# sheepTnT/Stage-IndexOrganized

Hardware: AMD Instinct MI355X
Metric: YCSB ops/sec at 1/2/4/8 GPU + achieved HBM GB/s vs peak; CPU ref ops/sec (higher is better)
Workload: dtype u64; 1 GPU; YCSB-C 100M rows uint64 keys, zipf 0.9, batched point-lookup on 1×MI355X; traversal=device, rows_per_gpu=100000000, rows_total=100000000, batch_per_gpu=16777216, key_bytes=8, payload_bytes=1000, leaf_bytes=65536, parallelism=single GPU

## Files before the change

stage-indexorganized_amd/csrc/capi.cpp:

```cpp
#include <hip/hip_runtime_api.h>

#include <execinfo.h>
#include <unistd.h>

#include <csignal>
#include <cstdlib>
#include <cstring>
#include <memory>
#include <stdexcept>
#include <string>
#include <vector>

#include "handle.hpp"

namespace stage_capi {
thread_local std::string g_err;
}
using namespace stage_capi;

extern "C" {

const char *stage_last_error(void) { return g_err.c_str(); }

namespace {
// ... 564 lines not shown
    if (rc) return rc;
    if (n && (!d_start_keys || !d_counts || (!d_records && scan_size))) return fail(STAGE_E_ARG, "null device buffer");
    hipError_t e = hipSetDevice(t->dev.device);
    if (e != hipSuccess) return hip_rc(e, "hipSetDevice");
    e = stage::launch_scan(t->dev.view, d_start_keys, d_lens, n, scan_size, d_counts, d_records, pick(t, stream),
                          t->scan_tune);
    return hip_rc(e, "scan kernel");
}

int stage_index_scan_batch(stage_table *t, const uint64_t *d_start_keys, const uint16_t *d_lens,
                           const uint32_t *d_read_ids, uint64_t n, uint32_t scan_size, uint32_t *d_counts,
                           uint8_t *d_records, uint8_t *d_row_status, void *stream) {
    int rc = need_synced(t);
    if (rc) return rc;
    if (n && (!d_start_keys || !d_counts || (scan_size && (!d_records || !d_row_status))))
        return fail(STAGE_E_ARG, "null device buffer");
    hipError_t e = hipSetDevice(t->dev.device);
    if (e != hipSuccess) return hip_rc(e, "hipSetDevice");
    e = stage::launch_scan(t->dev.view, d_start_keys, d_lens, n, scan_size, d_counts, d_records, pick(t, stream),
                           t->scan_tune, d_read_ids, d_row_status);
    return hip_rc(e, "index scan kernel");
}

static int scan_window(stage_table *t, const uint64_t *d_start_keys, const uint16_t *d_lens, const uint32_t *d_read_ids,
                       uint64_t n, uint32_t scan_size, uint32_t payload_off, uint32_t len, uint32_t *d_counts,
                       uint8_t *d_window, uint8_t *d_row_keys, uint8_t *d_row_status, bool index, void *stream) {
    int rc = check_window(t, payload_off, len);
    if (rc) return rc;
    if (n && scan_size && (!d_start_keys || !d_counts || !d_window || (index && !d_row_status)))
        return fail(STAGE_E_ARG, "null device buffer");
    rc = need_synced(t);
    if (rc) return rc;
    if (n == 0) return STAGE_OK;
    hipError_t e = hipSetDevice(t->dev.device);
    if (e != hipSuccess) return hip_rc(e, "hipSetDevice");
    e = stage::launch_scan_window(t->dev.view, d_start_keys, d_lens, n, scan_size, facts(t).key_pad() + payload_off, len,
                                  facts(t).key_pad(), d_counts, d_window, d_row_keys, pick(t, stream), t->scan_tune,
                                  index ? d_read_ids : nullptr, index ? d_row_status : nullptr);
    return hip_rc(e, index ? "window index scan kernel" : "window scan kernel");
}

int stage_scan_batch_window(stage_table *t, const uint64_t *d_start_keys, const uint16_t *d_lens, uint64_t n,
                            uint32_t scan_size, uint32_t payload_off, uint32_t len, uint32_t *d_counts,
                            uint8_t *d_window, uint8_t *d_row_keys, void *stream) {
    return scan_window(t, d_start_keys, d_lens, nullptr, n, scan_size, payload_off, len, d_counts, d_window, d_row_keys,
                       nullptr, false, stream);
}

int stage_index_scan_batch_window(stage_table *t, const uint64_t *d_start_keys, const uint16_t *d_lens,
                                  const uint32_t *d_read_ids, uint64_t n, uint32_t scan_size, uint32_t payload_off,
                                  uint32_t len, uint32_t *d_counts, uint8_t *d_window, uint8_t *d_row_keys,
                                  uint8_t *d_row_status, void *stream) {
    return scan_window(t, d_start_keys, d_lens, d_read_ids, n, scan_size, payload_off, len, d_counts, d_window,
                       d_row_keys, d_row_status, true, stream);
}

static int table_scan(stage_table *t, uint64_t leaf_begin, uint64_t leaf_end, const uint32_t *read_id, bool window,
                      uint32_t payload_off, uint32_t len, uint64_t max_records, uint64_t *d_count,
                      uint64_t *d_leaf_offsets, uint8_t *d_out, uint8_t *d_row_keys, uint64_t *d_row_meta,
                      uint8_t *d_row_status, void *stream) {
    if (!t) return fail(STAGE_E_ARG, "null table");
    int rc = window ? check_window(t, payload_off, len) : STAGE_OK;
    if (rc) return rc;
    if (leaf_begin > leaf_end) return fail(STAGE_E_ARG, "table scan: leaf_begin exceeds leaf_end");
    if (!d_count) return fail(STAGE_E_ARG, "table scan: null d_count");
    if (max_records && !d_out) return fail(STAGE_E_ARG, "table scan: null record buffer with max_records != 0");
    rc = need_synced(t);
    if (rc) return rc;
    const uint64_t nleaves = t->dev.view.nleaves;
    if (leaf_end == UINT64_MAX) leaf_end = nleaves;
    if (leaf_end > nleaves || leaf_begin > leaf_end)
        return fail(STAGE_E_ARG, "table scan: the leaf range exceeds the table's " + std::to_string(nleaves) + " leaves");
    return guarded([&] {
        hipError_t e = hipSetDevice(t->dev.device);
        if (e != hipSuccess) return hip_rc(e, "hipSetDevice");
        const uint32_t nl = (uint32_t)(leaf_end - leaf_begin);
        uint8_t *scratch = nl ? stage::scratch_bytes(t->dev, stage::table_scan_scratch_bytes(nl)) : nullptr;
        const stage::TableScanOut o{max_records, d_count, d_leaf_offsets, window ? nullptr : d_out,
                                    window ? d_out : nullptr, window ? d_row_keys : nullptr, d_row_meta, d_row_status};
        e = stage::launch_table_scan(t->dev.view, (uint32_t)leaf_begin, nl, read_id != nullptr, read_id ? *read_id : 0u,
                                     window ? facts(t).key_pad() + payload_off : 0u, window ? len : 0u,
                                     facts(t).key_pad(), o, scratch, pick(t, stream), t->scan_tune);
        return hip_rc(e, "table scan kernels");
    });
}

int stage_table_scan(stage_table *t, uint64_t leaf_begin, uint64_t leaf_end, const uint32_t *read_id,
                     uint64_t max_records, uint64_t *d_count, uint64_t *d_leaf_offsets, uint8_t *d_records,
                     uint64_t *d_row_meta, uint8_t *d_row_status, void *stream) {
    return table_scan(t, leaf_begin, leaf_end, read_id, false, 0, 0, max_records, d_count, d_leaf_offsets, d_records,
                      nullptr, d_row_meta, d_row_status, stream);
}

int stage_table_scan_window(stage_table *t, uint64_t leaf_begin, uint64_t leaf_end, const uint32_t *read_id,
                            uint32_t payload_off, uint32_t len, uint64_t max_records, uint64_t *d_count,
                            uint64_t *d_leaf_offsets, uint8_t *d_window, uint8_t *d_row_keys, uint64_t *d_row_meta,
                            uint8_t *d_row_status, void *stream) {
    return table_scan(t, leaf_begin, leaf_end, read_id, true, payload_off, len, max_records, d_count, d_leaf_offsets,
                      d_window, d_row_keys, d_row_meta, d_row_status, stream);
}

int stage_index_scan_first_batch(stage_table *t, const uint64_t *d_start_keys, const uint32_t *d_read_ids,
                                 uint64_t n, uint32_t scan_size, uint32_t prefix_words, uint32_t *d_image,
                                 uint8_t *d_status, void *stream) {
    int rc = need_synced(t);
    if (rc) return rc;
    if (t->dev.view.key_width == 0) return fail(STAGE_E_ARG, "first-tuple scans need fixed-width keys");
    if (scan_size == 0 || scan_size > 63) return fail(STAGE_E_ARG, "scan_size must be 1..63");
    if (prefix_words > t->dev.view.key_words) return fail(STAGE_E_ARG, "prefix_words exceeds the key's words");
    if (n && (!d_start_keys || !d_image || !d_status)) return fail(STAGE_E_ARG, "null device buffer");
    hipError_t e = hipSetDevice(t->dev.device);
    if (e != hipSuccess) return hip_rc(e, "hipSetDevice");
    e = stage::launch_scan_first(t->dev.view, d_start_keys, n, scan_size, d_read_ids, prefix_words, d_image, d_status,
                                 pick(t, stream), t->scan_tune);
    return hip_rc(e, "first-tuple scan kernel");
}

int stage_resolve_batch(stage_table *t, const uint64_t *d_keys, const uint16_t *d_lens, uint64_t n, int le_child,
                        uint32_t *d_leaf, void *stream) {
    int rc = need_synced(t);
    if (rc) return rc;
    if (n && (!d_keys || !d_leaf)) return fail(STAGE_E_ARG, "null device buffer");
    hipError_t e = hipSetDevice(t->dev.device);
    if (e != hipSuccess) return hip_rc(e, "hipSetDevice");
    e = stage::launch_resolve(t->dev.view, d_keys, d_lens, n, le_child, d_leaf, pick(t, stream));
    return hip_rc(e, "resolve kernel");
}

int stage_set_probe_tuning(stage_table *t, int group, int max_blocks) {
    if (!t || (group != 1 && group != 2 && group != 4 && group != 8) || max_blocks < 0)
        return fail(STAGE_E_ARG, "bad tuning");
    t->tune.group = group;
    t->tune.max_blocks = max_blocks;
    return STAGE_OK;
}

int stage_set_scan_tuning(stage_table *t, int max_blocks) {
    if (!t || max_blocks < 0) return fail(STAGE_E_ARG, "bad tuning");
    t->scan_tune.max_blocks = max_blocks;
    return STAGE_OK;
}

int stage_set_probe_store(stage_table *t, int policy) {
    if (!t || policy < STAGE_STORE_TEMPORAL || policy > STAGE_STORE_WRITE_THROUGH)
        return fail(STAGE_E_ARG, "bad store policy");
    t->tune.store = policy;
    return STAGE_OK;
}

int stage_set_probe_form(stage_table *t, int form) {
    if (!t || (form != STAGE_PROBE_FORM_WAVE && form != STAGE_PROBE_FORM_LANE))
        return fail(STAGE_E_ARG, "bad probe form");
    t->tune.form = form;
    return STAGE_OK;
}

int stage_murmur64a_batch(const void *d_keys, uint32_t key_len, uint32_t key_stride, uint64_t seed, uint64_t n,
                          uint64_t *d_out, void *stream) {
    if (n && (!d_keys || !d_out || key_stride < key_len)) return fail(STAGE_E_ARG, "bad arguments");
    return hip_rc(stage::launch_murmur(d_keys, key_len, key_stride, seed, n, d_out, (hipStream_t)stream),
                  "murmur kernel");
}

int stage_set_device(int device) { return hip_rc(hipSetDevice(device), "hipSetDevice"); }
int stage_device_count(int *count) { return hip_rc(hipGetDeviceCount(count), "hipGetDeviceCount"); }
int stage_dev_alloc(uint64_t bytes, void **ptr) { return hip_rc(hipMalloc(ptr, bytes ? bytes : 16), "hipMalloc"); }
int stage_dev_free(void *ptr) { return hip_rc(hipFree(ptr), "hipFree"); }
int stage_dev_memset(void *ptr, int value, uint64_t bytes, void *stream) {
    return hip_rc(hipMemsetAsync(ptr, value, bytes, (hipStream_t)stream), "hipMemsetAsync");
}
int stage_memcpy_h2d(void *dst, const void *src, uint64_t bytes, void *stream) {
    hipError_t e = hipMemcpyAsync(dst, src, bytes, hipMemcpyHostToDevice, (hipStream_t)stream);
    if (e == hipSuccess) e = hipStreamSynchronize((hipStream_t)stream);
    return hip_rc(e, "h2d");
}
int stage_memcpy_d2h(void *dst, const void *src, uint64_t bytes, void *stream) {
    hipError_t e = hipMemcpyAsync(dst, src, bytes, hipMemcpyDeviceToHost, (hipStream_t)stream);
    if (e == hipSuccess) e = hipStreamSynchronize((hipStream_t)stream);
    return hip_rc(e, "d2h");
}
int stage_stream_create(void **stream) {
    return hip_rc(hipStreamCreateWithFlags((hipStream_t *)stream, hipStreamNonBlocking), "hipStreamCreate");
}
int stage_stream_destroy(void *stream) { return hip_rc(hipStreamDestroy((hipStream_t)stream), "hipStreamDestroy"); }
int stage_stream_sync(void *stream) { return hip_rc(hipStreamSynchronize((hipStream_t)stream), "hipStreamSynchronize"); }
int stage_device_sync(void) { return hip_rc(hipDeviceSynchronize(), "hipDeviceSynchronize"); }
int stage_event_create(void **ev) { return hip_rc(hipEventCreate((hipEvent_t *)ev), "hipEventCreate"); }
int stage_event_destroy(void *ev) { return hip_rc(hipEventDestroy((hipEvent_t)ev), "hipEventDestroy"); }
int stage_event_record(void *ev, void *stream) {
    return hip_rc(hipEventRecord((hipEvent_t)ev, (hipStream_t)stream), "hipEventRecord");
}
int stage_event_elapsed(void *a, void *b, float *ms) {
    hipError_t e = hipEventSynchronize((hipEvent_t)b);
    if (e == hipSuccess) e = hipEventElapsedTime(ms, (hipEvent_t)a, (hipEvent_t)b);
    return hip_rc(e, "hipEventElapsedTime");
}

int stage_comm_unique_id(uint8_t *id128) {
    if (!id128) return fail(STAGE_E_ARG, "null argument");
    return guarded([&] { return stage::shard_unique_id(id128); });
}

int stage_comm_init(stage_table *t, const uint8_t *id128, int rank, int world) {
    if (!t || !id128 || world < 1 || rank < 0 || rank >= world) return fail(STAGE_E_ARG, "bad arguments");
    if (facts(t).key_words() != 1) return fail(STAGE_E_ARG, "the sharded front-end routes keys of <= 8 bytes");
    return guarded([&] {
        (void)hipSetDevice(t->dev.device);
        t->comm = std::make_unique<stage::ShardComm>();
        const int rc = stage::shard_init(*t->comm, id128, rank, world, t->shard_chunks);
        if (t->shard_dedupe >= 0) t->comm->dedupe = t->shard_dedupe != 0;
        t->comm->key_bits = t->shard_key_bits;
        return rc;
    });
}

int stage_set_shard_dedupe(stage_table *t, int on) {
    if (!t || on < -1 || on > 1) return fail(STAGE_E_ARG, "dedupe must be -1, 0 or 1");
    t->shard_dedupe = on;
    const bool v = on < 0 ? stage::shard_default_dedupe() : on != 0;
    if (t->comm) t->comm->dedupe = v;
    if (t->loop_comm) t->loop_comm->dedupe = v;
    return STAGE_OK;
}

int stage_set_write_overlap(stage_table *t, int on) {
    if (!t || on < 0 || on > 1) return fail(STAGE_E_ARG, "write overlap must be 0 or 1");
    t->wp_overlap = on;
    return STAGE_OK;
}

int stage_set_shard_key_bits(stage_table *t, int bits) {
    if (!t || bits < 0 || bits > 64) return fail(STAGE_E_ARG, "bits must be 0..64");
    t->shard_key_bits = bits ? bits : 64;
    if (t->comm) t->comm->key_bits = t->shard_key_bits;
    if (t->loop_comm) t->loop_comm->key_bits = t->shard_key_bits;
    return STAGE_OK;
}

int stage_rccl_info(int *runtime_version, int *header_version, char *path, uint64_t path_len) {
    return guarded([&] { return stage::shard_rccl_info(runtime_version, header_version, path, path_len); });
}

int stage_sharded_stats(stage_table *t, int loopback, uint64_t *n_keys, uint64_t *n_routed, uint64_t *n_remote) {
    if (!t || !n_keys || !n_routed || !n_remote) return fail(STAGE_E_ARG, "null argument");
    stage::ShardComm *c = loopback ? t->loop_comm.get() : t->comm.get();
    if (!c) return fail(STAGE_E_STATE, "no sharded probe has run");
    *n_keys = c->last_n;
    *n_routed = c->last_routed;
    *n_remote = c->last_remote;
    return STAGE_OK;
}

int stage_sharded_stats_ex(stage_table *t, int loopback, uint64_t *v, int nv) {
    if (!t || !v || nv < 0) return fail(STAGE_E_ARG, "bad arguments");
    stage::ShardComm *c = loopback ? t->loop_comm.get() : t->comm.get();
    if (!c) return fail(STAGE_E_STATE, "no sharded probe has run");
    const uint64_t all[4] = {c->last_n, c->last_routed, c->last_remote, c->last_received};
    for (int i = 0; i < nv && i < 4; ++i) v[i] = all[i];
    return STAGE_OK;
}

int stage_comm_allreduce_f64(stage_table *t, double *values, uint64_t n, int op) {
    if (!t || (!values && n) || op < 0 || op > 2) return fail(STAGE_E_ARG, "bad arguments");
    if (!t->comm) return fail(STAGE_E_STATE, "stage_comm_init first");
    return guarded([&] {
        (void)hipSetDevice(t->dev.device);
        return stage::shard_allreduce_f64(*t->comm, values, n, op);
    });
}

int stage_comm_allgather_f64(stage_table *t, const double *in, uint64_t n, double *out) {
    if (!t || ((!in || !out) && n)) return fail(STAGE_E_ARG, "bad arguments");
    if (!t->comm) return fail(STAGE_E_STATE, "stage_comm_init first");
    return guarded([&] {
        (void)hipSetDevice(t->dev.device);
        return stage::shard_allgather_f64(*t->comm, in, n, out);
    });
}

int stage_set_shard_chunks(stage_table *t, int chunks) {
    if (!t || chunks < 0 || chunks > 64) return fail(STAGE_E_ARG, "chunks must be 0..64");
    t->shard_chunks = chunks;
    return STAGE_OK;
}

int stage_comm_destroy(stage_table *t) {
    if (!t) return fail(STAGE_E_ARG, "null table");
    return guarded([&] {
        t->comm.reset();
        return STAGE_OK;
    });
}

int stage_probe_sharded(stage_table *t, const uint64_t *d_keys, const uint32_t *d_read_ids, uint64_t n,
                        stage_probe_out *d_out, uint8_t *d_records, void *stream) {
    int rc = need_synced(t);
    if (rc) return rc;
    if (!t->comm) return fail(STAGE_E_STATE, "stage_comm_init first");
    return guarded([&] {
        (void)hipSetDevice(t->dev.device);
        stage::DevTable view = t->dev.view;
        if (t->out_stride) view.stride = t->out_stride;
        return stage::shard_probe(*t->comm, view, t->tune, d_keys, d_read_ids, n,
                                  reinterpret_cast<stage::stage_probe_out_dev *>(d_out), d_records, STAGE_REPLY_ROWS,
                                  pick(t, stream));
    });
// ... 84 lines not shown
```

stage-indexorganized_amd/csrc/kernel_api.hpp:

```cpp
#pragma once
#include <hip/hip_runtime_api.h>

#include <cstdint>

#include "stage_core.hpp"

namespace stage {

struct alignas(16) stage_probe_out_dev {
    uint32_t w[8];
};

struct alignas(8) ImageDescDev {
    uint64_t key_le;
    uint64_t arg;
    uint32_t kind;
    uint32_t mode;
};

constexpr int kProbeFormWave = 0, kProbeFormLane = 1;
struct ProbeTuning {
    int group = 8;
    int max_blocks = 0;
    int store = 1;
    int status_bytes = 32;
    int form = kProbeFormLane;
};
constexpr int kProbeRows = 16;

hipError_t launch_resolve(const DevTable &t, const uint64_t *keys, const uint16_t *lens, uint64_t n, int le_child,
                          uint32_t *out, hipStream_t s);
hipError_t launch_probe(const DevTable &t, const uint64_t *keys, const uint16_t *lens, const uint32_t *rids,
                        const uint32_t *leaf_in, uint64_t n, stage_probe_out_dev *out, uint8_t *recs, hipStream_t s,
                        const ProbeTuning &tune, const uint64_t *d_n = nullptr, uint64_t shape_n = 0);
hipError_t launch_probe_window(const DevTable &t, const uint64_t *keys, const uint16_t *lens, const uint32_t *rids,
                               const uint32_t *leaf_in, uint64_t n, uint32_t row_off, uint32_t len,
                               stage_probe_out_dev *out, uint8_t *win, hipStream_t s, const ProbeTuning &tune);
bool probe_missed_supported(const DevTable &t);
hipError_t launch_probe_missed(const DevTable &t, const uint64_t *keys, uint64_t n, stage_probe_out_dev *out,
                               hipStream_t s, const ProbeTuning &tune, const uint64_t *d_n, uint64_t shape_n,
                               const uint32_t *mrids, uint32_t mnq, int32_t *missed);
struct alignas(8) FanRange {
    uint32_t lo, hi;
};
constexpr int kFanDests = 64;
struct FanDest {
    uint32_t nseg;
    uint32_t end[kFanDests];
    stage_probe_out_dev *out[kFanDests];
    uint8_t *recs[kFanDests];
};
bool probe_fanout_supported(const DevTable &t);
hipError_t launch_probe_fanout(const DevTable &t, const uint64_t *keys, const uint32_t *rids, uint64_t n,
                               const FanRange *fan, const uint32_t *flist, stage_probe_out_dev *out, uint8_t *recs,
                               hipStream_t s, const ProbeTuning &tune, const FanDest *dest = nullptr);
struct ScanTuning {
    int max_blocks = 0;
};

hipError_t launch_scan(const DevTable &t, const uint64_t *keys, const uint16_t *lens, uint64_t n, uint32_t scan_size,
                       uint32_t *counts, uint8_t *recs, hipStream_t s, const ScanTuning &tune,
                       const uint32_t *rids = nullptr, uint8_t *row_status = nullptr);
hipError_t launch_scan_window(const DevTable &t, const uint64_t *keys, const uint16_t *lens, uint64_t n,
                              uint32_t scan_size, uint32_t row_off, uint32_t len, uint32_t key_pad, uint32_t *counts,
                              uint8_t *win, uint8_t *row_keys, hipStream_t s, const ScanTuning &tune,
                              const uint32_t *rids = nullptr, uint8_t *row_status = nullptr);
struct TableScanOut {
    uint64_t max_records;
    uint64_t *count;
    uint64_t *leaf_offsets;
    uint8_t *recs;
    uint8_t *win;
    uint8_t *row_keys;
    uint64_t *row_meta;
    uint8_t *row_status;
};
uint64_t table_scan_scratch_bytes(uint64_t nl);
hipError_t launch_table_scan(const DevTable &t, uint32_t leaf0, uint32_t nl, bool snapshot, uint32_t rid,
                             uint32_t row_off, uint32_t len, uint32_t key_pad, const TableScanOut &o, uint8_t *scratch,
                             hipStream_t s, const ScanTuning &tune);
hipError_t launch_scan_pair(const DevTable &t0, const uint64_t *k0, uint32_t sz0, uint32_t *c0, uint8_t *r0,
                            const DevTable &t1, const uint64_t *k1, uint32_t sz1, uint32_t *c1, uint8_t *r1,
                            hipStream_t s);
bool scan_pair_supported(const DevTable &t0, uint32_t sz0, const DevTable &t1, uint32_t sz1);
hipError_t launch_scan_first(const DevTable &t, const uint64_t *keys, uint64_t n, uint32_t scan_size,
                             const uint32_t *rids, uint32_t words, uint32_t *img_out, uint8_t *st_out, hipStream_t s,
                             const ScanTuning &tune);
struct alignas(16) ReaderReq {
    uint64_t key;
    uint32_t rid;
    uint32_t tag;
};
struct ReaderRing {
    const ReaderReq *req;
    uint32_t *done;
    stage_probe_out_dev *out;
    uint8_t *rows;
    const uint32_t *stop;
    uint64_t *pos;
    uint32_t slots;
    uint32_t waves;
    uint64_t life_ticks;
    uint32_t *ident;
};
hipError_t launch_resident_reader(const DevTable &t, const ReaderRing &g, hipStream_t s);
hipError_t launch_revisit(const DevTable &t, const stage_probe_out_dev *base, uint64_t n, const uint32_t *rids,
                          uint32_t nq, const uint32_t *perm, stage_probe_out_dev *out, hipStream_t s,
                          const uint64_t *d_n = nullptr);
hipError_t launch_revisit_segments(const DevTable &t, const stage_probe_out_dev *base, uint64_t n,
                                   const uint64_t *seg_off, const uint32_t *seg_cnt, uint32_t nseg,
                                   const uint32_t *rids, uint32_t nq, stage_probe_out_dev *last, int32_t *missed,
                                   hipStream_t s, const uint64_t *d_n = nullptr, const uint64_t *d_nseg = nullptr);
hipError_t launch_for_update(const DevTable &t, const uint8_t *fu, const uint32_t *rids, uint64_t n,
                             stage_probe_out_dev *out, uint8_t *recs, hipStream_t s);
hipError_t launch_ident(const DevTable &t, const stage_probe_out_dev *out, uint64_t n, uint32_t *ident, hipStream_t s);
hipError_t launch_murmur(const void *keys, uint32_t key_len, uint32_t key_stride, uint64_t seed, uint64_t n,
                         uint64_t *out, hipStream_t s);
hipError_t launch_fill(uint8_t *heap, uint32_t stride, uint32_t payload_size, uint32_t row_bytes,
                       const ImageDescDev *descs, const uint8_t *arena, uint64_t first, uint64_t count,
                       uint64_t ident_rowid0, uint32_t ident_key_width, int ident_mode, hipStream_t s);
hipError_t launch_patch(uint8_t *head, uint64_t *okey, SlotInfo *slot, uint32_t head_bytes, uint32_t cap, uint32_t kw,
                        const uint32_t *head_leaf, const void *head_src, uint64_t nhead, const uint64_t *slot_idx,
                        const SlotInfo *slot_src, const uint64_t *words, uint64_t nslot, hipStream_t s);

}
```

stage-indexorganized_amd/csrc/probe.hip:

```cpp
#include <algorithm>

#include "kernel_api.hpp"
#include "launch_util.hpp"
#include "row_store.hpp"
#include "tree_search.hpp"

namespace stage {

template <int KW>
__global__ __launch_bounds__(256) void resolve_kernel(DevTable t, const uint64_t *__restrict__ keys,
                                                      const uint16_t *__restrict__ lens, uint64_t n, int le_child,
                                                      uint32_t *__restrict__ out) {
    uint64_t i = (uint64_t)blockIdx.x * blockDim.x + threadIdx.x;
    if (i >= n) return;
    uint32_t len = t.key_width ? t.key_width : (lens ? lens[i] : 8u);
    uint64_t ok[KW];
    load_okey<KW>(keys, i, true, len, ok);
    out[i] = t.key_width ? resolve_leaf<false, KW>(t, ok, len, le_child != 0)
                         : resolve_leaf<true, 1>(t, ok, len, le_child != 0);
}


template <bool VARLEN, int SPL, int G, int POL = 1, int ST = 32, bool FAN = false, bool DEST = false>
__global__ __launch_bounds__(256) void probe_kernel(DevTable t, const uint64_t *__restrict__ keys,
// ... 638 lines not shown
#pragma unroll
        for (int q = 0; q < SPL * 4; ++q) hv[q] = valid ? hp[q] : u32x4{0, 0, 0, 0};
        uint32_t c0 = 0, c1 = 0, c2 = 0, nc = 0;
#pragma unroll
        for (int q = 0; q < SPL * 4; ++q) {
            const uint32_t wq[4] = {hv[q].x, hv[q].y, hv[q].z, hv[q].w};
#pragma unroll
            for (int e = 0; e < 4; ++e) {
                const uint32_t w = wq[e] ^ rep;
                uint32_t zm = ~(((w & 0x7F7F7F7Fu) + 0x7F7F7F7Fu) | w) & 0x80808080u;
                while (zm) {
                    const uint32_t sl = (uint32_t)(q * 16 + e * 4) + ((uint32_t)__builtin_ctz(zm) >> 3);
                    c0 = nc == 0 ? sl : c0;
                    c1 = nc == 1 ? sl : c1;
                    c2 = nc == 2 ? sl : c2;
                    ++nc;
                    zm &= zm - 1;
                }
            }
        }
        if (!valid) nc = 0;
        int slot = -1;
        uint64_t m = 0;
        uint32_t nx = 0, im = 0;
        const uint64_t lb = (uint64_t)leaf * t.cap;
        auto confirm = [&](uint32_t sl) { return confirm_slot<KW>(t, leaf, lb, sl, ok, slot, m, nx, im); };
        if (nc > 0) confirm(c0);
        if (slot < 0 && nc > 1) confirm(c1);
        if (slot < 0 && nc > 2) confirm(c2);
        if (slot < 0 && nc > 3) {
            const uint8_t *h = t.head + (uint64_t)leaf * t.head_bytes;
            const uint8_t fx = (uint8_t)rep;
            for (uint32_t sl = c2 + 1; sl < t.cap; ++sl)
                if (h[sl] == fx && confirm(sl)) break;
        }
        ProbeRes r;
        visibility(t, slot, m, nx, im, rid, r);
        if (MISS && valid)
            for (uint32_t q = 0; q < mnq; ++q) {
                ProbeRes rq;
                visibility(t, slot, m, nx, im, mrids[q], rq);
                if (rq.status != ST_LATEST && rq.status != ST_COPY && rq.status != ST_OLD) atomicOr(missed + q, 1);
            }
        store_chunk(t, lane, base, (int)((n - base) < 64 ? (n - base) : 64), valid, leaf, r, out, recs, out_chunks);
    }
}

template <int SPL, int R, int ST>
__global__ __launch_bounds__(256) void probe_rows_kernel(DevTable t, const uint64_t *__restrict__ keys,
                                                         const uint32_t *__restrict__ rids,
                                                         const uint32_t *__restrict__ leaf_in, uint64_t n,
                                                         stage_probe_out_dev *__restrict__ out,
                                                         uint8_t *__restrict__ recs) {
    static_assert(SPL <= 2, "probe_kernel's leaves: 64 or 128 slots");
    const uint32_t lane = lane_id();
    const uint64_t wave = (uint64_t)blockIdx.x * (blockDim.x >> 6) + uni32(threadIdx.x >> 6);
    const uint64_t nwaves = (uint64_t)gridDim.x * (blockDim.x >> 6);
    const uint32_t out_chunks = t.stride >> 4;
    const uint32_t len = t.key_width;
    for (uint64_t base = wave * 64; base < n; base += nwaves * 64) {
        const uint64_t i = base + lane;
        const bool valid = i < n;
        const uint32_t rid = rids ? (valid ? rids[i] : 0u) : 0xFFFFFFFEu;
        uint64_t ok;
        load_okey<1>(keys, i, valid, len, &ok);
        uint32_t leaf = 0;
        if (valid) leaf = leaf_in ? leaf_in[i] : resolve_leaf<false, 1>(t, &ok, len, true);
        if (leaf > t.nseps) leaf = t.nseps;
        const uint32_t rep = (key_fp_words(&ok, 1) & 0xFFu) * 0x01010101u;
        u32x4 hv[SPL * 4];
        const u32x4 *hp = reinterpret_cast<const u32x4 *>(t.head + (uint64_t)leaf * t.head_bytes);
#pragma unroll
        for (int q = 0; q < SPL * 4; ++q) hv[q] = valid ? hp[q] : u32x4{0, 0, 0, 0};
        uint32_t c0 = 0, c1 = 0, c2 = 0, nc = 0;
#pragma unroll
        for (int q = 0; q < SPL * 4; ++q) {
            const uint32_t wq[4] = {hv[q].x, hv[q].y, hv[q].z, hv[q].w};
#pragma unroll
            for (int e = 0; e < 4; ++e) {
                const uint32_t w = wq[e] ^ rep;
                uint32_t zm = ~(((w & 0x7F7F7F7Fu) + 0x7F7F7F7Fu) | w) & 0x80808080u;
                while (zm) {
                    const uint32_t sl = (uint32_t)(q * 16 + e * 4) + ((uint32_t)__builtin_ctz(zm) >> 3);
                    c0 = nc == 0 ? sl : c0;
                    c1 = nc == 1 ? sl : c1;
                    c2 = nc == 2 ? sl : c2;
                    ++nc;
                    zm &= zm - 1;
                }
            }
        }
        if (!valid) nc = 0;
        int slot = -1;
        uint64_t m = 0;
        uint32_t nx = 0, im = 0;
        const uint64_t lb = (uint64_t)leaf * t.cap;
        auto confirm = [&](uint32_t sl) { return confirm_slot<1>(t, leaf, lb, sl, &ok, slot, m, nx, im); };
        if (nc > 0) confirm(c0);
        if (slot < 0 && nc > 1) confirm(c1);
        if (slot < 0 && nc > 2) confirm(c2);
        if (slot < 0 && nc > 3) {
            const uint8_t *h = t.head + (uint64_t)leaf * t.head_bytes;
            const uint8_t fx = (uint8_t)rep;
            for (uint32_t sl = c2 + 1; sl < t.cap; ++sl)
                if (h[sl] == fx && confirm(sl)) break;
        }
        ProbeRes r;
        if (slot >= 0 && !meta_inserting(m) && rid >= meta_cstamp(m) && (nx & kNextKindMask) != kNextCopy) {
            r.status = ST_LATEST;
            r.flags = 0;
            r.hops = 0;
            r.slot = (uint32_t)slot;
            r.meta_hi = (uint32_t)(m >> 32);
            r.cstamp = rid;
            r.rec_cstamp = meta_cstamp(m);
            r.copy_sstamp = kMaxCid;
            r.image = im;
        } else {
            visibility(t, slot, m, nx, im, rid, r);
        }
        if (valid) {
            u32x4 a, b;
            pack_out(leaf, r, a, b);
            if constexpr (ST == 16) {
                st16<1>(u32x4{a.x, a.w, b.y, b.x}, reinterpret_cast<uint8_t *>(out) + base * 16u, lane * 16u);
            } else {
                uint8_t *ob = reinterpret_cast<uint8_t *>(out + base);
                st16<1>(a, ob, lane * 32u);
                st16<1>(b, ob, lane * 32u + 16u);
            }
        }
        if (!recs) continue;
        const int cnt = (int)((n - base) < 64 ? (n - base) : 64);
        for (int j0 = 0; j0 < cnt; j0 += R) {
            for (uint32_t k0 = 0; k0 < out_chunks; k0 += 64) {
                const uint32_t c = k0 + lane;
                u32x4 v[R];
#pragma unroll
                for (int g = 0; g < R; ++g) {
                    const uint32_t img = rl32(r.image, j0 + g < cnt ? j0 + g : cnt - 1);
                    v[g] = u32x4{0, 0, 0, 0};
                    if (c < out_chunks && img != 0xFFFFFFFFu) v[g] = heap_chunk(t, img, c);
                }
#pragma unroll
                for (int g = 0; g < R; ++g) {
                    const int j = j0 + g;
                    if (j < cnt && c < out_chunks) st16<1>(v[g], recs + (base + j) * (uint64_t)t.stride, c * 16u);
                }
            }
        }
    }
}


hipError_t launch_resolve(const DevTable &t, const uint64_t *keys, const uint16_t *lens, uint64_t n, int le_child,
                          uint32_t *out, hipStream_t s) {
    if (n == 0) return hipSuccess;
    const unsigned b = (unsigned)((n + 255) / 256);
    with_key_words(t, [&](auto KW) { resolve_kernel<KW()><<<b, 256, 0, s>>>(t, keys, lens, n, le_child, out); });
    return hipGetLastError();
}

constexpr uint64_t kSmallBelow = 16384;

hipError_t launch_probe(const DevTable &t, const uint64_t *keys, const uint16_t *lens, const uint32_t *rids,
                        const uint32_t *leaf_in, uint64_t n, stage_probe_out_dev *out, uint8_t *recs, hipStream_t s,
                        const ProbeTuning &tune, const uint64_t *d_n, uint64_t shape_n) {
    if (n == 0) return hipSuccess;
    if (d_n) {
        if (!(t.key_words > 1 || (t.key_width != 0 && t.cap > 128))) return hipErrorInvalidValue;
    }
    const int mb = max_blocks(tune);
    const int blocks = grid_for((n + 63) / 64, 4, mb);
    const bool var = t.key_width == 0;
    if (t.key_words > 1 || (!var && t.cap > 128)) {
        const uint64_t sn = d_n && shape_n ? std::min(shape_n, n) : n;
        const bool small = (sn + 63) / 64 < (uint64_t)kSmallBelow;
        const bool tiny = (sn + 15) / 16 < (uint64_t)kSmallBelow / 4;
        with_geometry(t, [&](auto S, auto KW) {
            if constexpr (S() <= 4) {
                probe_lane_kernel<S(), KW()><<<grid_for((sn + 63) / 64, 4, mb), 256, 0, s>>>(t, keys, rids, leaf_in, n,
                                                                                             out, recs, d_n);
            } else if (tiny) {
                probe_split_kernel<S(), KW(), 4><<<grid_for((sn + 3) / 4, 4, mb), 256, 0, s>>>(t, keys, rids, leaf_in, n,
                                                                                               out, recs, d_n);
            } else if (small) {
                probe_split_kernel<S(), KW(), 16><<<grid_for((sn + 15) / 16, 4, mb), 256, 0, s>>>(t, keys, rids, leaf_in,
                                                                                                  n, out, recs, d_n);
            } else {
                probe_split_kernel<S(), KW(), 64><<<blocks, 256, 0, s>>>(t, keys, rids, leaf_in, n, out, recs, d_n);
            }
        });
        return hipGetLastError();
    }
    if (!var && tune.form == kProbeFormLane && tune.group == 8 && tune.store == 1 &&
        (tune.status_bytes != 16 || t.cap == 64)) {
        auto launch_rows = [&](auto kernel) { kernel<<<blocks, 256, 0, s>>>(t, keys, rids, leaf_in, n, out, recs); };
        if (tune.status_bytes == 16) launch_rows(probe_rows_kernel<1, kProbeRows, 16>);
        else if (t.cap == 64) launch_rows(probe_rows_kernel<1, kProbeRows, 32>);
        else launch_rows(probe_rows_kernel<2, kProbeRows, 32>);
        return hipGetLastError();
    }
    auto launch = [&](auto kernel) {
        kernel<<<blocks, 256, 0, s>>>(t, keys, lens, rids, leaf_in, n, out, recs, nullptr, nullptr, nullptr);
    };
    if (tune.status_bytes == 16) {
        if (var || t.cap != 64 || tune.group != 8 || tune.store != 1) return hipErrorInvalidValue;
        launch(probe_kernel<false, 1, 8, 1, 16>);
        return hipGetLastError();
    }
    if (t.cap == 64) {
        if (var) launch(probe_kernel<true, 1, 4>);
        else if (tune.group == 1) launch(probe_kernel<false, 1, 1>);
        else if (tune.group == 2) launch(probe_kernel<false, 1, 2>);
        else if (tune.group == 4) launch(probe_kernel<false, 1, 4>);
        else if (tune.store == 0) launch(probe_kernel<false, 1, 8, 0>);
        else if (tune.store == 2) launch(probe_kernel<false, 1, 8, 2>);
        else launch(probe_kernel<false, 1, 8>);
    } else {
        if (var) launch(probe_kernel<true, 2, 4>);
        else launch(probe_kernel<false, 2, 4>);
    }
    return hipGetLastError();
}

hipError_t launch_probe_window(const DevTable &t, const uint64_t *keys, const uint16_t *lens, const uint32_t *rids,
                               const uint32_t *leaf_in, uint64_t n, uint32_t row_off, uint32_t len,
                               stage_probe_out_dev *out, uint8_t *win, hipStream_t s, const ProbeTuning &tune) {
    if (len == 0 || (uint64_t)row_off + len > t.hstride || (n && !win)) return hipErrorInvalidValue;
    if (n == 0) return hipSuccess;
    const WindowArgs w{row_off, len, (len + 15u) >> 4, win};
    const int mb = max_blocks(tune);
    const int blocks = grid_for((n + 63) / 64, 4, mb);
    const bool var = t.key_width == 0;
    if (t.key_words > 1 || (!var && t.cap > 128)) {
        ProbeTuning full = tune;
        full.status_bytes = 32;
        const hipError_t e = launch_probe(t, keys, lens, rids, leaf_in, n, out, nullptr, s, full);
        if (e != hipSuccess) return e;
        window_gather_kernel<<<blocks, 256, 0, s>>>(t, out, n, w);
        return hipGetLastError();
    }
    if (tune.status_bytes == 16 && (var || t.cap != 64)) return hipErrorInvalidValue;
    hipError_t e = hipErrorInvalidValue;
    with_slot_groups(t, [&](auto S) {
        if constexpr (S() <= 2) {
            auto launch = [&](auto kernel) {
                kernel<<<blocks, 256, 0, s>>>(t, keys, lens, rids, leaf_in, n, out, w);
                e = hipGetLastError();
            };
            if (var) {
                launch(probe_window_kernel<true, S(), 4, 32>);
            } else if constexpr (S() == 1) {
                if (tune.status_bytes == 16) launch(probe_window_kernel<false, 1, 8, 16>);
                else launch(probe_window_kernel<false, 1, 8, 32>);
            } else {
                launch(probe_window_kernel<false, 2, 4, 32>);
            }
        }
    });
    return e;
}

hipError_t launch_probe_missed(const DevTable &t, const uint64_t *keys, uint64_t n, stage_probe_out_dev *out,
                               hipStream_t s, const ProbeTuning &tune, const uint64_t *d_n, uint64_t shape_n,
                               const uint32_t *mrids, uint32_t mnq, int32_t *missed) {
    if (!probe_missed_supported(t)) return hipErrorInvalidValue;
    if (n == 0) return hipSuccess;
    const uint64_t sn = d_n && shape_n ? std::min(shape_n, n) : n;
    const int blocks = grid_for((sn + 63) / 64, 4, max_blocks(tune));
    with_geometry(t, [&](auto S, auto KW) {
        if constexpr (S() <= 4)
            probe_lane_kernel<S(), KW(), true><<<blocks, 256, 0, s>>>(t, keys, nullptr, nullptr, n, out, nullptr, d_n,
                                                                      mrids, mnq, missed);
    });
    return hipGetLastError();
}

bool probe_missed_supported(const DevTable &t) {
    const bool wide = t.key_words > 1 || (t.key_width != 0 && t.cap > 128);
    return wide && t.key_width != 0 && t.cap <= 256 && (t.cap == 64 || t.cap == 128 || t.cap == 256);
}

hipError_t launch_probe_fanout(const DevTable &t, const uint64_t *keys, const uint32_t *rids, uint64_t n,
                               const FanRange *fan, const uint32_t *flist, stage_probe_out_dev *out, uint8_t *recs,
                               hipStream_t s, const ProbeTuning &tune, const FanDest *dest) {
    if (!probe_fanout_supported(t)) return hipErrorInvalidValue;
    if (n == 0) return hipSuccess;
    if ((!recs && !dest) || (!fan && !flist)) return hipErrorInvalidValue;
    const int blocks = grid_for((n + 63) / 64, 4, max_blocks(tune));
    if (dest)
        probe_kernel<false, 1, 4, 1, 32, true, true><<<blocks, 256, 0, s>>>(t, keys, nullptr, rids, nullptr, n, out,
                                                                            recs, fan, flist, dest);
    else
        probe_kernel<false, 1, 8, 1, 32, true><<<blocks, 256, 0, s>>>(t, keys, nullptr, rids, nullptr, n, out, recs,
                                                                      fan, flist);
    return hipGetLastError();
}

bool probe_fanout_supported(const DevTable &t) {
    return t.key_width != 0 && t.key_words == 1 && t.cap == 64 && t.stride <= 1024;
}

__global__ __launch_bounds__(256) void revisit_kernel(DevTable t, const stage_probe_out_dev *__restrict__ base,
                                                      uint64_t n, const uint32_t *__restrict__ rids, uint32_t nq,
                                                      const uint32_t *__restrict__ perm,
                                                      stage_probe_out_dev *__restrict__ out,
                                                      const uint64_t *__restrict__ dn) {
    if (dn) n = *dn < n ? *dn : n;
    const uint64_t g = (uint64_t)blockIdx.x * blockDim.x + threadIdx.x;
    if (g >= n * nq) return;
    const uint64_t i = g % n, q = g / n;
    const u32x4 *bp = reinterpret_cast<const u32x4 *>(base + i);
    u32x4 a = bp[0], b = bp[1];
    revisit_one(t, rids[q], a, b);
    u32x4 *op = reinterpret_cast<u32x4 *>(out + q * n + (perm ? perm[i] : i));
    op[0] = a;
    op[1] = b;
}

constexpr uint32_t kRevisitQ = 16;
__global__ __launch_bounds__(256) void revisit_missed_kernel(DevTable t, const stage_probe_out_dev *__restrict__ base,
                                                             uint64_t n, const uint32_t *__restrict__ rids, uint32_t nq,
                                                             int32_t *__restrict__ missed, const uint64_t *__restrict__ dn) {
    if (dn) n = *dn < n ? *dn : n;
    const uint64_t g = (uint64_t)blockIdx.x * blockDim.x + threadIdx.x;
    if (g >= n * ((nq + kRevisitQ - 1) / kRevisitQ)) return;
    const uint64_t i = g % n;
    const uint32_t q0 = (uint32_t)(g / n) * kRevisitQ, q1 = q0 + kRevisitQ < nq ? q0 + kRevisitQ : nq;
    const u32x4 *bp = reinterpret_cast<const u32x4 *>(base + i);
    const u32x4 a0 = bp[0];
    const uint32_t slot = a0.z & 0xFFFF, leaf = a0.y;
    const bool redo = (a0.x & 0xFF) != ST_NOT_FOUND && slot < t.cap && leaf < t.nleaves;
    SlotInfo si = {};
    if (redo) si = t.slot[(uint64_t)leaf * t.cap + slot];
    for (uint32_t q = q0; q < q1; ++q) {
        uint32_t st = a0.x & 0xFF;
        if (redo) {
            ProbeRes r;
            visibility(t, (int)slot, si.meta, si.next, si.image, rids[q], r);
            st = r.status;
        }
        if (st != ST_LATEST && st != ST_COPY && st != ST_OLD) atomicOr(missed + q, 1);
    }
}

__global__ __launch_bounds__(256) void revisit_last_kernel(DevTable t, const stage_probe_out_dev *__restrict__ base,
                                                           const uint64_t *__restrict__ seg_off,
                                                           const uint32_t *__restrict__ seg_cnt, uint32_t nseg,
                                                           const uint32_t *__restrict__ rids, uint32_t nq,
                                                           stage_probe_out_dev *__restrict__ last,
                                                           const uint64_t *__restrict__ dseg) {
    if (dseg) nseg = *dseg < nseg ? (uint32_t)*dseg : nseg;
    const uint64_t g = (uint64_t)blockIdx.x * blockDim.x + threadIdx.x;
    if (g >= (uint64_t)nseg * nq) return;
    const uint32_t k = (uint32_t)(g % nseg), q = (uint32_t)(g / nseg);
    const uint32_t c = seg_cnt[k];
    if (c == 0) return;
    const u32x4 *bp = reinterpret_cast<const u32x4 *>(base + seg_off[k] + c - 1);
    u32x4 a = bp[0], b = bp[1];
    revisit_one(t, rids[q], a, b);
    u32x4 *op = reinterpret_cast<u32x4 *>(last + g);
    op[0] = a;
    op[1] = b;
}

hipError_t launch_revisit_segments(const DevTable &t, const stage_probe_out_dev *base, uint64_t n,
                                   const uint64_t *seg_off, const uint32_t *seg_cnt, uint32_t nseg,
                                   const uint32_t *rids, uint32_t nq, stage_probe_out_dev *last, int32_t *missed,
                                   hipStream_t s, const uint64_t *d_n, const uint64_t *d_nseg) {
    if (nq == 0) return hipSuccess;
    const uint64_t tm = n * ((nq + kRevisitQ - 1) / kRevisitQ), tl = (uint64_t)nseg * nq;
    if (tm) revisit_missed_kernel<<<(unsigned)((tm + 255) / 256), 256, 0, s>>>(t, base, n, rids, nq, missed, d_n);
    if (tl)
        revisit_last_kernel<<<(unsigned)((tl + 255) / 256), 256, 0, s>>>(t, base, seg_off, seg_cnt, nseg, rids, nq, last,
                                                                         d_nseg);
    return hipGetLastError();
}

hipError_t launch_revisit(const DevTable &t, const stage_probe_out_dev *base, uint64_t n, const uint32_t *rids,
                          uint32_t nq, const uint32_t *perm, stage_probe_out_dev *out, hipStream_t s,
                          const uint64_t *d_n) {
    if (n == 0 || nq == 0) return hipSuccess;
    revisit_kernel<<<(unsigned)((n * nq + 255) / 256), 256, 0, s>>>(t, base, n, rids, nq, perm, out, d_n);
    return hipGetLastError();
}

__global__ __launch_bounds__(256) void ident_kernel(DevTable t, const stage_probe_out_dev *__restrict__ out, uint64_t n,
                                                    uint32_t *__restrict__ ident) {
    const uint64_t i = (uint64_t)blockIdx.x * blockDim.x + threadIdx.x;
    if (i >= n) return;
    const u32x4 a = reinterpret_cast<const u32x4 *>(out + i)[0];
    const uint32_t status = a.x & 0xFF, leaf = a.y, slot = a.z & 0xFFFF;
    uint32_t loc = 0, next = 0;
    if (status != ST_NOT_FOUND && slot < t.cap && leaf < t.nleaves) {
        const u32x4 w1 = reinterpret_cast<const u32x4 *>(t.slot + (uint64_t)leaf * t.cap + slot)[1];
        next = w1.x;
        loc = w1.z;
    }
    reinterpret_cast<uint2 *>(ident)[i] = make_uint2(loc, next);
}

__global__ __launch_bounds__(256) void for_update_kernel(DevTable t, const uint8_t *__restrict__ fu,
                                                         const uint32_t *__restrict__ rids, uint64_t n,
                                                         stage_probe_out_dev *__restrict__ out, uint8_t *__restrict__ recs) {
    const uint32_t lane = lane_id();
    const uint64_t base = ((uint64_t)blockIdx.x * (blockDim.x >> 6) + uni32(threadIdx.x >> 6)) * 64;
    const uint64_t i = base + lane;
    uint64_t todo = ballot(i < n && fu[i] != 0);
    const uint32_t chunks = t.stride >> 4;
    while (todo) {
        const int j = __builtin_ctzll(todo);
        todo &= todo - 1;
        const uint64_t p = base + (uint64_t)j;
        const u32x4 *op = reinterpret_cast<const u32x4 *>(out + p);
        u32x4 a = op[0], b = op[1];
        const uint32_t rid = rids ? rids[p] : 0xFFFFFFFEu;
        const uint32_t slot = a.z & 0xFFFF, leaf = a.y;
        uint32_t image = 0xFFFFFFFFu;
        if (slot < t.cap && leaf < t.nleaves) {
            const SlotInfo si = t.slot[(uint64_t)leaf * t.cap + slot];
            ProbeRes r;
            visibility<true>(t, (int)slot, si.meta, si.next, si.image, rid, r);
            pack_out(leaf, r, a, b);
            image = r.image;
        } else {
            a.x |= 2u << 8;
        }
        if (lane < 2) reinterpret_cast<u32x4 *>(out + p)[lane] = lane == 0 ? a : b;
        if (recs) {
            for (uint32_t c = lane; c < chunks; c += 64) {
                u32x4 v = u32x4{0, 0, 0, 0};
                if (image != 0xFFFFFFFFu) v = heap_chunk(t, image, c);
                reinterpret_cast<u32x4 *>(recs + p * (uint64_t)t.stride)[c] = v;
            }
        }
    }
}

hipError_t launch_for_update(const DevTable &t, const uint8_t *fu, const uint32_t *rids, uint64_t n,
                             stage_probe_out_dev *out, uint8_t *recs, hipStream_t s) {
    if (n == 0) return hipSuccess;
    for_update_kernel<<<(unsigned)((n + 255) / 256), 256, 0, s>>>(t, fu, rids, n, out, recs);
// ... 22 lines not shown
```

Baseline: 2.818 billion ops/s.

## Add lane-per-key fanout probe kernel with wave-cooperative record copy

```diff
diff --git a/stage-indexorganized_amd/csrc/capi.cpp b/stage-indexorganized_amd/csrc/capi.cpp
--- a/stage-indexorganized_amd/csrc/capi.cpp
+++ b/stage-indexorganized_amd/csrc/capi.cpp
@@ -740,6 +740,7 @@
     if (!t || (form != STAGE_PROBE_FORM_WAVE && form != STAGE_PROBE_FORM_LANE))
         return fail(STAGE_E_ARG, "bad probe form");
     t->tune.form = form;
+    t->tune.fan_form = form;
     return STAGE_OK;
 }
 
diff --git a/stage-indexorganized_amd/csrc/kernel_api.hpp b/stage-indexorganized_amd/csrc/kernel_api.hpp
--- a/stage-indexorganized_amd/csrc/kernel_api.hpp
+++ b/stage-indexorganized_amd/csrc/kernel_api.hpp
@@ -19,14 +19,18 @@
 };
 
 constexpr int kProbeFormWave = 0, kProbeFormLane = 1;
+constexpr int kFanFormAuto = -1;
 struct ProbeTuning {
     int group = 8;
     int max_blocks = 0;
     int store = 1;
     int status_bytes = 32;
     int form = kProbeFormLane;
+    int fan_form = kFanFormAuto;
 };
 constexpr int kProbeRows = 16;
+constexpr int kFanRows = 16, kFanRowsDest = 8;
+constexpr bool kFanOwnStatus = true;
 
 hipError_t launch_resolve(const DevTable &t, const uint64_t *keys, const uint16_t *lens, uint64_t n, int le_child,
                           uint32_t *out, hipStream_t s);
diff --git a/stage-indexorganized_amd/csrc/probe.hip b/stage-indexorganized_amd/csrc/probe.hip
--- a/stage-indexorganized_amd/csrc/probe.hip
+++ b/stage-indexorganized_amd/csrc/probe.hip
@@ -814,6 +814,152 @@
     }
 }
 
+template <int R, bool DEST, bool OWN>
+__global__ __launch_bounds__(256) void probe_fan_kernel(DevTable t, const uint64_t *__restrict__ keys,
+                                                        const uint32_t *__restrict__ rids, uint64_t n,
+                                                        stage_probe_out_dev *__restrict__ out,
+                                                        uint8_t *__restrict__ recs, const FanRange *__restrict__ fan,
+                                                        const uint32_t *__restrict__ flist,
+                                                        const FanDest *__restrict__ dest) {
+    const uint32_t lane = lane_id();
+    __shared__ uint32_t s_dend[DEST ? kFanDests : 1];
+    __shared__ stage_probe_out_dev *s_dout[DEST ? kFanDests : 1];
+    __shared__ uint8_t *s_drec[DEST ? kFanDests : 1];
+    uint32_t nseg = 0;
+    if constexpr (DEST) {
+        nseg = dest->nseg;
+        for (uint32_t g = threadIdx.x; g < nseg; g += blockDim.x)
+            s_dend[g] = dest->end[g], s_dout[g] = dest->out[g], s_drec[g] = dest->recs[g];
+        __syncthreads();
+    }
+    const uint64_t wave = (uint64_t)blockIdx.x * (blockDim.x >> 6) + uni32(threadIdx.x >> 6);
+    const uint64_t nwaves = (uint64_t)gridDim.x * (blockDim.x >> 6);
+    const uint32_t out_chunks = t.stride >> 4;
+    const uint32_t len = t.key_width;
+    for (uint64_t base = wave * 64; base < n; base += nwaves * 64) {
+        const uint64_t i = base + lane;
+        const bool valid = i < n;
+        const uint32_t rid = rids ? (valid ? rids[i] : 0u) : 0xFFFFFFFEu;
+        FanRange my_fan = FanRange{0u, 0u};
+        if (valid) my_fan = fan ? fan[i] : FanRange{(uint32_t)i, (uint32_t)i + 1u};
+        uint64_t my_o = (uint64_t)out, my_r = (uint64_t)recs;
+        if constexpr (DEST) {
+            uint32_t sg = 0;
+            for (uint32_t g = 0; g + 1 < nseg; ++g) sg += i >= s_dend[g] ? 1u : 0u;
+            my_o = (uint64_t)s_dout[sg];
+            my_r = (uint64_t)s_drec[sg];
+        }
+        uint32_t pos0 = 0;
+        if (OWN && my_fan.hi > my_fan.lo) pos0 = flist ? flist[my_fan.lo] : my_fan.lo;
+        uint64_t ok;
+        load_okey<1>(keys, i, valid, len, &ok);
+        uint32_t leaf = 0;
+        if (valid) leaf = resolve_leaf<false, 1>(t, &ok, len, true);
+        if (leaf > t.nseps) leaf = t.nseps;
+        const uint32_t rep = (key_fp_words(&ok, 1) & 0xFFu) * 0x01010101u;
+        u32x4 hv[4];
+        const u32x4 *hp = reinterpret_cast<const u32x4 *>(t.head + (uint64_t)leaf * t.head_bytes);
+#pragma unroll
+        for (int q = 0; q < 4; ++q) hv[q] = valid ? hp[q] : u32x4{0, 0, 0, 0};
+        uint32_t c0 = 0, c1 = 0, c2 = 0, nc = 0;
+#pragma unroll
+        for (int q = 0; q < 4; ++q) {
+            const uint32_t wq[4] = {hv[q].x, hv[q].y, hv[q].z, hv[q].w};
+#pragma unroll
+            for (int e = 0; e < 4; ++e) {
+                const uint32_t w = wq[e] ^ rep;
+                uint32_t zm = ~(((w & 0x7F7F7F7Fu) + 0x7F7F7F7Fu) | w) & 0x80808080u;
+                while (zm) {
+                    const uint32_t sl = (uint32_t)(q * 16 + e * 4) + ((uint32_t)__builtin_ctz(zm) >> 3);
+                    c0 = nc == 0 ? sl : c0;
+                    c1 = nc == 1 ? sl : c1;
+                    c2 = nc == 2 ? sl : c2;
+                    ++nc;
+                    zm &= zm - 1;
+                }
+            }
+        }
+        if (!valid) nc = 0;
+        int slot = -1;
+        uint64_t m = 0;
+        uint32_t nx = 0, im = 0;
+        const uint64_t lb = (uint64_t)leaf * t.cap;
+        auto confirm = [&](uint32_t sl) { return confirm_slot<1>(t, leaf, lb, sl, &ok, slot, m, nx, im); };
+        if (nc > 0) confirm(c0);
+        if (slot < 0 && nc > 1) confirm(c1);
+        if (slot < 0 && nc > 2) confirm(c2);
+        if (slot < 0 && nc > 3) {
+            const uint8_t *h = t.head + (uint64_t)leaf * t.head_bytes;
+            const uint8_t fx = (uint8_t)rep;
+            for (uint32_t sl = c2 + 1; sl < t.cap; ++sl)
+                if (h[sl] == fx && confirm(sl)) break;
+        }
+        ProbeRes r;
+        if (slot >= 0 && !meta_inserting(m) && rid >= meta_cstamp(m) && (nx & kNextKindMask) != kNextCopy) {
+            r.status = ST_LATEST;
+            r.flags = 0;
+            r.hops = 0;
+            r.slot = (uint32_t)slot;
+            r.meta_hi = (uint32_t)(m >> 32);
+            r.cstamp = rid;
+            r.rec_cstamp = meta_cstamp(m);
+            r.copy_sstamp = kMaxCid;
+            r.image = im;
+        } else {
+            visibility(t, slot, m, nx, im, rid, r);
+        }
+        u32x4 a, b;
+        pack_out(leaf, r, a, b);
+        if (OWN && my_fan.hi > my_fan.lo) {
+            uint8_t *ob = reinterpret_cast<uint8_t *>(reinterpret_cast<stage_probe_out_dev *>(my_o) + pos0);
+            st16<1>(a, ob, 0u);
+            st16<1>(b, ob, 16u);
+        }
+        const int cnt = (int)((n - base) < 64 ? (n - base) : 64);
+        for (int j0 = 0; j0 < cnt; j0 += R) {
+            u32x4 v[R];
+            uint32_t mine0[R];
+#pragma unroll
+            for (int g = 0; g < R; ++g) {
+                const int j = j0 + g < cnt ? j0 + g : cnt - 1;
+                const uint32_t img = rl32(r.image, j);
+                v[g] = u32x4{0, 0, 0, 0};
+                if (lane < out_chunks && img != 0xFFFFFFFFu) v[g] = heap_chunk(t, img, lane);
+                const uint32_t lo = rl32(my_fan.lo, j), hi = rl32(my_fan.hi, j);
+                const uint32_t kk = lo + lane;
+                mine0[g] = j0 + g < cnt && kk < hi ? (flist ? flist[kk] : kk) : 0u;
+            }
+#pragma unroll
+            for (int g = 0; g < R; ++g) {
+                const int j = j0 + g;
+                if (j >= cnt) break;
+                const uint32_t lo = rl32(my_fan.lo, j), hi = rl32(my_fan.hi, j);
+                stage_probe_out_dev *o_j = reinterpret_cast<stage_probe_out_dev *>(rl64(my_o, j));
+                uint8_t *r_j = reinterpret_cast<uint8_t *>(rl64(my_r, j));
+                uint32_t k = 0;
+                if constexpr (OWN) {
+                    if (hi > lo && lane < out_chunks)
+                        st16<1>(v[g], r_j + rl32(mine0[g], 0) * (uint64_t)t.stride, lane * 16u);
+                    if (hi - lo <= 1u) continue;
+                    k = 1;
+                }
+                const u32x4 half = lane == 0 ? u32x4{rl32(a.x, j), rl32(a.y, j), rl32(a.z, j), rl32(a.w, j)}
+                                             : u32x4{rl32(b.x, j), rl32(b.y, j), rl32(b.z, j), rl32(b.w, j)};
+                for (uint32_t k0 = lo; k0 < hi; k0 += 64, k = 0) {
+                    const uint32_t kk = k0 + lane;
+                    const uint32_t mine = k0 == lo ? mine0[g] : kk < hi ? (flist ? flist[kk] : kk) : 0u;
+                    const uint32_t kn = hi - k0 < 64u ? hi - k0 : 64u;
+                    for (; k < kn; ++k) {
+                        const uint64_t pos = rl32(mine, (int)k);
+                        if (lane < out_chunks) st16<1>(v[g], r_j + pos * (uint64_t)t.stride, lane * 16u);
+                        if (lane < 2) st16<1>(half, reinterpret_cast<uint8_t *>(o_j + pos), lane * 16u);
+                    }
+                }
+            }
+        }
+    }
+}
+
 
 hipError_t launch_resolve(const DevTable &t, const uint64_t *keys, const uint16_t *lens, uint64_t n, int le_child,
                           uint32_t *out, hipStream_t s) {
@@ -951,6 +1097,16 @@
     if (n == 0) return hipSuccess;
     if ((!recs && !dest) || (!fan && !flist)) return hipErrorInvalidValue;
     const int blocks = grid_for((n + 63) / 64, 4, max_blocks(tune));
+    const bool lane = tune.fan_form == kFanFormAuto ? !dest && !flist : tune.fan_form == kProbeFormLane;
+    if (lane) {
+        if (dest)
+            probe_fan_kernel<kFanRowsDest, true, kFanOwnStatus><<<blocks, 256, 0, s>>>(t, keys, rids, n, out, recs, fan,
+                                                                                       flist, dest);
+        else
+            probe_fan_kernel<kFanRows, false, kFanOwnStatus><<<blocks, 256, 0, s>>>(t, keys, rids, n, out, recs, fan,
+                                                                                    flist, nullptr);
+        return hipGetLastError();
+    }
     if (dest)
         probe_kernel<false, 1, 4, 1, 32, true, true><<<blocks, 256, 0, s>>>(t, keys, nullptr, rids, nullptr, n, out,
                                                                             recs, fan, flist, dest);
```

Result: slower. 2.764 billion ops/s (-1.9%).
